# jarrodhroberson/diamond-types

Measured on AMD Instinct MI355X. Metric: merged ops/sec (whole node) for batched checkout, higher is better.
Workload: dtype u32/u8 integer

## Files before the change

diamond-types_amd/csrc/dt_device.hpp:

```cpp
#pragma once
#include <hip/hip_runtime.h>
#include <stdint.h>
#include <cstdio>

#include "dt_host.hpp"

namespace dtgpu {

inline hipError_t launch_error(const char *file = __builtin_FILE(), int line = __builtin_LINE()) {
    const hipError_t e = hipGetLastError();
    if (e != hipSuccess) fprintf(stderr, "[dtgpu] launch error at %s:%d: %s\n", file, line, hipGetErrorString(e));
    return e;
}

struct DocDesc {
    uint64_t cmd_off;
    uint64_t lv_off;
    uint64_t content_off;
    uint64_t arun_off;
    uint64_t blk_off;
    uint64_t out_off;
    uint64_t gidx_off;
    uint64_t tlist_off;
    uint32_t ncmd, n_lv, n_aruns, max_blocks, out_cap, content_len;
    uint32_t ascii;
    uint32_t seg_lo, seg_hi, seg_u, src_cap;
    uint64_t pc_off;
    uint64_t src_off;
    uint32_t flags;
};
constexpr uint32_t SEG_PHANTOM = 0x80000000u;
constexpr uint32_t DOC_CRITICAL = 1u;
constexpr uint32_t DOC_FF = 2u;
constexpr uint32_t DOC_CUT_HOST = 4u;

struct DocResult {
    uint32_t status, out_len;
    uint64_t hash;
    uint32_t n_items, n_blocks;
    uint32_t fail_cmd, fail_site;
    uint32_t n_sb, lds;
    uint32_t dbg[22];
};

constexpr uint32_t LOC_CNT_SHIFT = 24;
constexpr uint32_t LOC_BLK_SHIFT = 6;
constexpr uint32_t LOC_BLK_MASK = 0x3FFFF;
constexpr uint32_t LOC_MAX_BLOCKS = LOC_BLK_MASK + 1;

struct BatchParams {
    const Cmd *cmds;
    const uint32_t *tlist;
    const uint32_t *cbyte;
    const uint8_t *content;
    const uint32_t *aruns;
    uint32_t *pos;
    unsigned long long *ao;
    uint32_t *items;
    unsigned long long *m2;
    uint8_t *out;
    uint8_t *gidx;
    const DocDesc *docs;
    const uint32_t *doc_list;
    uint32_t n_list;
    uint32_t lds_blocks;
// ... 113 lines not shown
```

diamond-types_amd/csrc/dt_replay.hip:

```cpp
#include <hip/hip_runtime.h>

#include <algorithm>
#include <cstdlib>
#include <stdint.h>

#include "dt_device.hpp"
#include "dt_wave.hpp"

namespace dtgpu {
namespace dev {
using namespace wave;

#define BALLOT(c) __ballot(c)
DEV uint32_t vflag(bool c) {
    uint32_t x = c ? 1u : 0u;
    asm volatile("" : "+v"(x));
    return x;
}

constexpr uint32_t BLK = 64;
constexpr uint32_t SBC = 64;
constexpr uint32_t ROOT_ID = 0xFFFFFFFFu;
constexpr uint32_t END_ID = 0xFFFFFFFEu;
constexpr uint32_t NONE = 0xFFFFFFFFu;
// ... 10 lines not shown

template <typename T> DEV T ld(const T *p) { return *p; }
template <typename T> DEV T vld(const T *p) { return *reinterpret_cast<const volatile T *>(p); }
DEV const BatchParams &KP() {
    return *(const BatchParams *)(__builtin_amdgcn_kernarg_segment_ptr());
}
#define GLOBAL_AS __attribute__((address_space(1)))
template <typename T> DEV GLOBAL_AS T *gp(T *p) { return (GLOBAL_AS T *)p; }
template <typename T> DEV void st(T *p, T v) { *p = v; }
template <typename T> DEV T ld_sc(const T *p) { return __hip_atomic_load(p, __ATOMIC_RELAXED, __HIP_MEMORY_SCOPE_WORKGROUP); }
template <typename T> DEV void st_sc(T *p, T v) { __hip_atomic_store(p, v, __ATOMIC_RELAXED, __HIP_MEMORY_SCOPE_WORKGROUP); }
DEV uint32_t cv_add(uint32_t *p, uint32_t d) { return __hip_atomic_fetch_add(p, d, __ATOMIC_RELAXED, __HIP_MEMORY_SCOPE_WORKGROUP); }
template <typename T> DEV void at_xor(T *p, T v) { __hip_atomic_fetch_xor(p, v, __ATOMIC_RELAXED, __HIP_MEMORY_SCOPE_WORKGROUP); }
template <typename T> DEV void at_add(T *p, T v) { __hip_atomic_fetch_add(p, v, __ATOMIC_RELAXED, __HIP_MEMORY_SCOPE_WORKGROUP); }
template <typename T> DEV void at_or(T *p, T v) { __hip_atomic_fetch_or(p, v, __ATOMIC_RELAXED, __HIP_MEMORY_SCOPE_WORKGROUP); }

template <int L> DEV uint32_t ix(const uint32_t *p) {
    if (L) return *p;
    return ld_sc(p);
}
template <int L> DEV uint32_t ix16(const uint16_t *p) { return *p; }

enum ProfSlot { P_INS = 0, P_DEL, P_TOG, P_MAT, P_YJS, P_SPLIT, P_FIND, P_BLOAD, P_ORR, P_RUN, P_R1, P_R2, P_R3, P_N_YJS, P_N_SPLIT,
                P_T1, P_T2, P_T3, P_N_DIRTY, P_N_LOAD, P_N };

struct Doc {
    const Cmd *cmds;
    uint32_t ncmd, n_lv;
    const uint32_t *tlist;
    const DocDesc *desc;
    uint32_t *pc;
    u64 *ao;
    uint32_t *items;
    u64 *m2;
    uint32_t max_blocks, max_sb;
    uint32_t *cnt, *opos;
    uint16_t *opos16;
    uint32_t *sbn, *sbpos;
    uint32_t *top, *tlive;
    uint16_t *sbl;
    uint32_t nb, nsb;
    uint32_t err;
    uint32_t debug;
    uint32_t site;
    uint32_t steps;
    uint64_t prof[P_N];
    uint32_t doc;
    uint32_t cb, cit;
    u64 cmv, cml;
    u64 *mup;
    uint32_t *tup;
    uint32_t *xf;
};

DEV void fail(Doc &D, uint32_t code, uint32_t site) {
    if (!D.err) { D.err = code; D.site = site; }
}
DEV bool charge(Doc &D) {
    if (D.steps == 0) { fail(D, ErrCapacity, 1); return false; }
    D.steps--;
    return true;
}
template <bool PROF> DEV uint64_t tick() { return PROF ? __builtin_amdgcn_s_memtime() : 0; }

constexpr int IX_HBM = 0, IX_LDS = 1, IX_FLAT = 2;
template <int L> DEV uint32_t opos_of(const Doc &D, uint32_t b) {
    if (L) return D.opos16[b];
    return ix<L>(D.opos + b);
}
template <int L> DEV void set_opos(Doc &D, uint32_t b, uint32_t v) {
    if (L) D.opos16[b] = uint16_t(v);
    else D.opos[b] = v;
}


template <int L> DEV uint32_t first_block(const Doc &D) {
// ... 29 lines not shown
            const uint32_t o = 4 * (q + uint32_t(j));
            if (v[j].w == item) s = o + 3;
            if (v[j].z == item) s = o + 2;
            if (v[j].y == item) s = o + 1;
            if (v[j].x == item) s = o;
        }
    }
    return s;
}
template <int L> DEV uint32_t key_of(const Doc &D, uint32_t item) {
    const uint32_t b = pc_blk(ld(D.pc + item));
    return key_at<L>(D, b, find_slot(D, b, item));
}
template <int L> DEV uint32_t ukey_of(const Doc &D, uint32_t item) {
    const uint32_t b = U(pc_blk(ld(D.pc + item)));
    const u64 m = BALLOT(D.items[size_t(b) * BLK + lane()] == item);
    return U(key_at<L>(D, b, ctz(m)));
}

struct Found {
    uint32_t b, k;
    uint32_t S, tp;
    uint32_t c;
};
template <int L>
DEV bool find_vis(Doc &D, uint32_t p, Found &f) {
    const uint32_t l = lane();
    uint32_t base = 0, S = NONE;
    if (L == IX_FLAT) {
        const uint32_t nc = (D.nb + 63) >> 6;
        {
            const uint32_t w0 = D.top[min(l, nc - 1)];
            const uint32_t v = l < nc ? (w0 & 0xFFFFu) : 0u;
            const uint32_t inc = scan_incl32(v);
            const u64 m = BALLOT(inc > p) & 0xFFFFFFFFull;
            if (!m) return false;
            S = ctz(m);
            base = rdl(inc - v, S);
        }
        f.S = f.tp = S;
        const uint32_t q = (S << 6) + l;
        const uint32_t b0 = D.sbl[min(q, D.nb - 1)];
        const uint32_t w = D.cnt[b0];
        const uint32_t b = q < D.nb ? b0 : 0;
        const uint32_t v = q < D.nb ? c_vis(w) : 0;
        const uint32_t inc = scan_incl(v);
        const u64 m = BALLOT(base + inc > p);
        if (!m) return false;
        const uint32_t fl = ctz(m);
        f.b = U(rdl(b, fl));
        f.k = U(p - base - rdl(inc - v, fl));
        f.c = U(rdl(w, fl));
        return true;
    }
    for (uint32_t c = 0; c < D.nsb; c += 64) {
        const uint32_t i = c + l;
        const uint32_t w0 = ix<L>(D.top + min(i, D.nsb - 1));
        const uint32_t w = i < D.nsb ? w0 : 0;
        const uint32_t v = w & 0xFFFFu;
        const uint32_t inc = scan_incl(v);
        const u64 m = BALLOT(base + inc > p);
        if (m) {
            const uint32_t fl = ctz(m);
            S = U(rdl(w, fl) >> 16);
            f.tp = U(c + fl);
            base += rdl(inc - v, fl);
            break;
        }
        base += rdl(inc, 63);
    }
    if (S == NONE) return false;
    f.S = S;
    f.c = NONE;
    const uint32_t n = U(ix<L>(D.sbn + S));
    const uint32_t b0 = ix16<L>(D.sbl + size_t(S) * SBC + l);
// ... 206 lines not shown
    D.nb++;
    if (n + 1 == SBC) split_sb<L, XF>(D, S);
    return b2;
}

template <int L> DEV uint32_t cut_point(uint32_t s) { return L ? min(max(s, 16u), 48u) : BLK / 2; }

template <int L>
DEV uint32_t up_rank(Doc &D, uint32_t b, uint32_t s) {
    const uint32_t l = lane();
    const uint32_t o = U(opos_of<L>(D, b));
    const uint32_t S = o >> 6, i = o & 63u, tp = U(ix<L>(D.sbpos + S));
    uint32_t r = 0;
    for (uint32_t c = 0; c < tp; c += 64) r += wave_sum(c + l < tp ? ix<L>(D.tup + c + l) : 0u);
    const uint32_t bl = l < i ? ix16<L>(D.sbl + size_t(S) * SBC + l) : 0;
    r += wave_sum(l < i ? c_up(ix<L>(D.cnt + bl)) : 0u);
    r += uint32_t(__popcll(U64(ld(D.mup + b)) & lanes_below(s)));
    return U(r);
}

template <int L, bool PROF, bool XF>
DEV void insert_run(Doc &D, uint32_t b, uint32_t s, uint32_t it, u64 mv, u64 ml, uint32_t lv, uint32_t k,
                    uint32_t ol, uint32_t orr, uint32_t tph, uint32_t c_in) {
    D.cb = NONE;
    const uint32_t l = lane();
    const uint32_t lv0 = lv, k0 = k;
    if (XF) {
        const uint32_t r0 = up_rank<L>(D, b, s);
        for (uint32_t j = l; j < k0; j += 64) D.xf[lv0 + j] = r0 + j;
    }
    if (!XF && c_in != NONE && c_items(c_in) + k <= BLK) {
        const uint32_t shifted = shfl(it, l >= k ? l - k : l);
        it = l < s ? it : (l < s + k ? lv + (l - s) : shifted);
        D.items[size_t(b) * BLK + l] = it;
        if (l >= s && l < s + k) st(D.pc + it, pc_of(b, 1u));
        const u64 low = lanes_below(s);
        const u64 ins = lanes_below(k) << s;
        mv = k == 64 ? ins : ((mv & low) | ((mv & ~low) << k) | ins);
        ml = k == 64 ? ins : ((ml & low) | ((ml & ~low) << k) | ins);
        st(D.m2 + 2 * size_t(b) + (l & 1u), (l & 1u) ? ml : mv);
        if (tph == NONE) tph = L == IX_FLAT ? U(uint32_t(D.opos16[b]) >> 6) : U(ix<L>(D.sbpos + (opos_of<L>(D, b) >> 6)));
        if (l == 0) {
            D.cnt[b] = c_in + k * (C_VIS + C_LIVE + C_ITEMS);
            if (L == IX_FLAT) {
                at_add(D.top + tph, k | (k << 16));
            } else {
                at_add(D.top + tph, k);
// ... 45 lines not shown
            u64 mu = U64(ld(D.mup + b));
            mu = m == 64 ? ins : ((mu & low) | ((mu & ~low) << m) | ins);
            if (l == 0) st(D.mup + b, mu);
        }
        if (tph == NONE) tph = L == IX_FLAT ? U(uint32_t(D.opos16[b]) >> 6) : U(ix<L>(D.sbpos + (opos_of<L>(D, b) >> 6)));
        if (l == 0) {
            D.cnt[b] = c + m * (C_VIS + C_LIVE + C_ITEMS + (XF ? C_UP : 0u));
            const uint32_t tp = tph;
            if (L == IX_FLAT) {
                at_add(D.top + tp, m | (m << 16));
            } else {
                at_add(D.top + tp, m);
                at_add(D.tlive + tp, m);
            }
            if (XF) at_add(D.tup + tp, m);
        }
        fence_wave();
        if (PROF) { const uint64_t t = tick<PROF>(); D.prof[P_R2] += t - tr; tr = t; }
        lv += m;
        k -= m;
        s += m;
    }
    D.cb = b; D.cit = it; D.cmv = mv; D.cml = ml;
    const uint64_t t3 = tick<PROF>();
    for (uint32_t j0 = 0; j0 < k0; j0 += 64) {
        const uint32_t j = j0 + l, nit = lv0 + j;
        if (j < k0) D.ao[nit] = u64(j == 0 ? ol : nit - 1) | (u64(orr) << 32);
    }
    if (PROF) D.prof[P_R3] += tick<PROF>() - t3;
}

DEV void agent_of(Doc &D, uint32_t lv, uint32_t &rank, uint32_t &seq) {
    const uint32_t l = lane();
    const GLOBAL_AS uint32_t *aruns = gp(vld(&KP().aruns)) + U(uint32_t(vld(&D.desc->arun_off)));
    uint32_t lo = 0, n = U(vld(&D.desc->n_aruns));
    while (n > 64) {
        if (!charge(D)) { rank = seq = 0; return; }
        const uint32_t stride = (n + 63) / 64;
        const uint32_t idx = lo + l * stride;
        const bool ok = l * stride < n && aruns[4 * idx] <= lv;
        const uint32_t k = uint32_t(__popcll(BALLOT(ok)));
        const uint32_t nlo = lo + (k ? k - 1 : 0) * stride;
        n = min(stride, lo + n - nlo);
        lo = nlo;
    }
    const bool ok = l < n && aruns[4 * (lo + l)] <= lv;
// ... 85 lines not shown
    const uint32_t bc = c_items(c);
    if (PROF) { D.prof[P_N_LOAD]++; if (c & C_DIRTY) D.prof[P_N_DIRTY]++; }
    const uint32_t it0 = D.items[size_t(b) * BLK + l];
    it = l < bc ? it0 : 0;
    if (c & C_DIRTY) {
        const uint32_t k = pc_cnt(ld(D.pc + it));
        mv = BALLOT(l < bc && k == 1u);
        ml = BALLOT(l < bc && k != 0u);
        st(D.m2 + 2 * size_t(b) + (l & 1u), (l & 1u) ? ml : mv);
        if (l == 0) D.cnt[b] = c & ~C_DIRTY;
        fence_wave();
    } else {
        const u64 x = ld(D.m2 + 2 * size_t(b) + (l & 1u));
        mv = rdl64(x, 0);
        ml = rdl64(x, 1);
    }
}

template <int L, bool PROF, bool XF>
DEV void do_insert(Doc &D, uint32_t lv, uint32_t k, uint32_t pos) {
    uint64_t tp = tick<PROF>();
    uint32_t b, kk = 0, tph = 0;
    uint32_t fcnt = NONE;
    if (pos == 0) {
        b = first_block<L>(D);
    } else {
        Found f;
        if (!find_vis<L>(D, pos - 1, f)) { fail(D, ErrCheckout, 13); return; }
        b = f.b;
        kk = f.k;
        tph = f.tp;
        fcnt = f.c;
    }
    if (PROF) { const uint64_t t = tick<PROF>(); D.prof[P_FIND] += t - tp; tp = t; }
    const uint32_t c0 = L == IX_FLAT && fcnt != NONE ? fcnt : U(ix<L>(D.cnt + b));
    const uint32_t bc = c_items(c0);
    uint32_t cb = c0 & ~C_DIRTY;
    uint32_t it;
    u64 mv, ml;
    if (b == D.cb) { it = D.cit; mv = D.cmv; ml = D.cml; }
    else load_block<L, PROF>(D, b, c0, it, mv, ml);
    uint32_t s = 0, ol = ROOT_ID;
    if (pos) {
        const uint32_t s0 = select_bit(mv, kk);
        if (s0 >= bc) { fail(D, ErrCheckout, 13); return; }
        ol = U(rdl(it, s0));
        s = s0 + 1;
    }
    if (PROF) { const uint64_t t = tick<PROF>(); D.prof[P_BLOAD] += t - tp; tp = t; }
    const u64 mlr = s >= 64 ? 0ull : (ml & (~0ull << s));
    uint32_t rb, rs, orr;
    bool direct;
    if (mlr) {
        rb = b;
        rs = ctz(mlr);
        orr = U(rdl(it, rs));
// ... 10 lines not shown
        } else {
            rs = 0;
            orr = END_ID;
        }
        if (s < bc) direct = false;
        else {
            const uint32_t nx = next_block<L>(D, b);
            direct = nx == NONE || (rb == nx && rs == 0);
        }
    }
    if (PROF) { const uint64_t t = tick<PROF>(); D.prof[P_ORR] += t - tp; tp = t; }
    if (!direct) {
        const uint32_t my_l = ol == ROOT_ID ? 0u : ukey_of<L>(D, ol) + 1u;
        const uint32_t my_r = orr == END_ID ? 0xFFFFFFFFu : ukey_of<L>(D, orr);
        const uint32_t b0 = b;
        yjs_scan<L>(D, b, s, rb, rs, my_l, my_r, ol, orr, lv);
        if (D.err) return;
        if (b != b0) {
            cb = U(ix<L>(D.cnt + b));
            if (b == D.cb) { it = D.cit; mv = D.cmv; ml = D.cml; }
            else load_block<L, PROF>(D, b, cb, it, mv, ml);
            cb &= ~C_DIRTY;
            tph = NONE;
        }
        if (PROF) { const uint64_t t = tick<PROF>(); D.prof[P_YJS] += t - tp; tp = t; D.prof[P_N_YJS]++; }
    }
    const uint64_t sp0 = PROF ? D.prof[P_SPLIT] : 0;
    insert_run<L, PROF, XF>(D, b, s, it, mv, ml, lv, k, ol, orr, tph, cb);
    if (PROF) D.prof[P_RUN] += tick<PROF>() - tp - (D.prof[P_SPLIT] - sp0);
}

template <int L, bool PROF, bool XF>
DEV void do_delete(Doc &D, uint32_t lv, uint32_t n, uint32_t pos, bool fwd) {
    const uint32_t l = lane();
    uint32_t j0 = 0;
    uint32_t up_done = 0;
    while (j0 < n) {
        Found f;
        if (!find_vis<L>(D, pos, f)) { fail(D, ErrCheckout, 14); return; }
        const uint32_t b = f.b, kk = f.k, tpos = f.tp;
        const uint32_t c0 = L == IX_FLAT && f.c != NONE ? f.c : U(ix<L>(D.cnt + b));
        uint32_t it;
        u64 mv, ml;
        if (b == D.cb) { it = D.cit; mv = D.cmv; ml = D.cml; }
        else load_block<L, PROF>(D, b, c0, it, mv, ml);
        const uint32_t c = c0 & ~C_DIRTY;
        const uint32_t avail = c_vis(c) - kk;
        const uint32_t take = min(avail, n - j0);
        const uint32_t r = uint32_t(__popcll(mv & lanes_below(l)));
        const bool sel = ((mv >> l) & 1ull) && r >= kk && r < kk + take;
        const u64 selm = BALLOT(sel);
        if (uint32_t(__popcll(selm)) != take || take == 0) { fail(D, ErrCheckout, 15); return; }
        u64 mu = 0;
        uint32_t base = 0;
        if (XF) {
            mu = U64(ld(D.mup + b));
            base = up_rank<L>(D, b, 0);
        }
        if (sel) {
            const uint32_t j = j0 + (r - kk);
            const uint32_t dlv = fwd ? lv + j : lv + n - 1 - j;
            st(D.pc + it, pc_of(b, 2u));
// ... 85 lines not shown
                    else act = false;
                }
            }
            dm &= ~same;
        }
        bool fv = false, fl = false;
        uint32_t b = 0;
        int32_t dv = 0, dl = 0;
        {
            const uint32_t w = ld(D.pc + (act ? item : 0u));
            const uint32_t bw = pc_blk(w), oc = pc_cnt(w), nc = oc + uint32_t(d);
            const bool badc = act && int32_t((oc + uint32_t(dneg)) | (0xFFFFu - nc) | (D.nb - 1u - bw)) < 0;
            const bool ok = act && !badc;
            bad = bad || badc;
            if (ok) st(D.pc + item, pc_of(bw, nc));
            b = ok ? bw : 0u;
            fv = ok && ((oc == 1) != (nc == 1));
            fl = ok && ((oc != 0) != (nc != 0));
            dv = fv ? (nc == 1 ? 1 : -1) : 0;
            dl = fl ? (nc != 0 ? 1 : -1) : 0;
        }
        if (BALLOT(bad)) { fail(D, ErrCheckout, 16); return; }
        const bool flip = fv || fl;
        if (BALLOT(flip && b == D.cb)) D.cb = NONE;
        if (PROF) { const uint64_t t = tick<PROF>(); D.prof[P_T2] += t - tq; tq = t; }
        if (L == IX_FLAT) {
            if (flip) {
                at_add(D.top + (uint32_t(D.opos16[b]) >> 6), uint32_t(dv) + (uint32_t(dl) << 16));
                at_add(D.cnt + b, uint32_t(dv) * C_VIS + uint32_t(dl) * C_LIVE);
                at_or(D.cnt + b, C_DIRTY);
            }
        } else if (L) {
            if (flip) {
                const uint32_t tp = ix<L>(D.sbpos + (opos_of<L>(D, b) >> 6));
                if (fv) at_add(D.top + tp, uint32_t(dv));
                if (fl) at_add(D.tlive + tp, uint32_t(dl));
                at_add(D.cnt + b, uint32_t(dv) * C_VIS + uint32_t(dl) * C_LIVE);
                at_or(D.cnt + b, C_DIRTY);
            }
        } else {
            for (u64 pend = BALLOT(flip); pend;) {
                const uint32_t f = ctz(pend);
                const uint32_t bb = rdl(b, f);
                const u64 same = BALLOT(flip && b == bb);
                const bool mine = (same >> l) & 1ull;
                const uint32_t sv = wave_sum(mine ? uint32_t(dv) : 0u), sl = wave_sum(mine ? uint32_t(dl) : 0u);
                if (l == f) {
                    const uint32_t tp = ix<L>(D.sbpos + (opos_of<L>(D, bb) >> 6));
                    if (sv) at_add(D.top + tp, sv);
                    if (sl) at_add(D.tlive + tp, sl);
                    at_add(D.cnt + bb, sv * C_VIS + sl * C_LIVE);
                    at_or(D.cnt + bb, C_DIRTY);
                }
                pend &= ~same;
// ... 49 lines not shown
                const int32_t sum = int32_t(wave_sum(mine ? uint32_t(d) : 0u));
                const int32_t neg = int32_t(wave_sum(mine ? uint32_t(dneg) : 0u));
                if (mine) {
                    if (l == ctz(same)) { d = sum; dneg = neg; }
                    else act = false;
                }
            }
            dm &= ~same;
        }
    }
    if (PROF) { const uint64_t t = tick<PROF>(); D.prof[P_T1] += t - tq; tq = t; }
    const uint32_t w = ld(D.pc + (act ? item : 0u));
    const uint32_t bw = pc_blk(w), oc = pc_cnt(w), nc = oc + uint32_t(d);
    const bool badc = act && int32_t((oc + uint32_t(dneg)) | (0xFFFFu - nc) | (D.nb - 1u - bw)) < 0;
    const bool ok = act && !badc;
    if (ok) st(D.pc + item, pc_of(bw, nc));
    if (BALLOT(bad || badc)) { fail(D, ErrCheckout, 16); return; }
    const uint32_t b = ok ? bw : 0u;
    const bool fv = ok && ((oc == 1) != (nc == 1));
    const bool fl = ok && ((oc != 0) != (nc != 0));
    const int32_t dv = fv ? (nc == 1 ? 1 : -1) : 0;
    const int32_t dl = fl ? (nc != 0 ? 1 : -1) : 0;
    const bool flip = fv || fl;
    if (BALLOT(flip && b == D.cb)) D.cb = NONE;
    if (PROF) { const uint64_t t = tick<PROF>(); D.prof[P_T2] += t - tq; tq = t; }
    if (L == IX_FLAT) {
        if (flip) {
            at_add(D.top + (uint32_t(D.opos16[b]) >> 6), uint32_t(dv) + (uint32_t(dl) << 16));
            at_add(D.cnt + b, uint32_t(dv) * C_VIS + uint32_t(dl) * C_LIVE);
            at_or(D.cnt + b, C_DIRTY);
        }
    } else if (L) {
        if (flip) {
            const uint32_t tp = ix<L>(D.sbpos + (opos_of<L>(D, b) >> 6));
            if (fv) at_add(D.top + tp, uint32_t(dv));
            if (fl) at_add(D.tlive + tp, uint32_t(dl));
            at_add(D.cnt + b, uint32_t(dv) * C_VIS + uint32_t(dl) * C_LIVE);
            at_or(D.cnt + b, C_DIRTY);
        }
    } else {
        for (u64 pend = BALLOT(flip); pend;) {
            const uint32_t f = ctz(pend);
            const uint32_t bb = rdl(b, f);
            const u64 same = BALLOT(flip && b == bb);
            const bool mine = (same >> l) & 1ull;
            const uint32_t sv = wave_sum(mine ? uint32_t(dv) : 0u), sl = wave_sum(mine ? uint32_t(dl) : 0u);
            if (l == f) {
                const uint32_t tp = ix<L>(D.sbpos + (opos_of<L>(D, bb) >> 6));
                if (sv) at_add(D.top + tp, sv);
                if (sl) at_add(D.tlive + tp, sl);
                at_add(D.cnt + bb, sv * C_VIS + sl * C_LIVE);
                at_or(D.cnt + bb, C_DIRTY);
            }
            pend &= ~same;
// ... 336 lines not shown
                    if (w != b || find_slot(D, b, it) != l) bad = true;
                }
            } else if (((mv | ml) >> l) & 1) bad = true;
            const u64 bm = BALLOT(bad);
            if (bm) {
                if (l == ctz(bm)) {
                    res->dbg[0] = b; res->dbg[1] = l; res->dbg[2] = cnt; res->dbg[3] = it; res->dbg[4] = w;
                    res->dbg[5] = uint32_t(mv); res->dbg[6] = uint32_t(mv >> 32);
                    res->dbg[7] = uint32_t(ml); res->dbg[8] = uint32_t(ml >> 32);
                }
                return 202;
            }
            blocks++;
        }
        if (tv != (U(ix<L>(D.top + p)) & 0xFFFFu)) return 203;
        if (tl != (L == IX_FLAT ? U(ix<L>(D.top + p)) >> 16 : U(ix<L>(D.tlive + p)))) return 204;
        if (XF && tu != U(ix<L>(D.tup + p))) return 210;
    }
    if (blocks != D.nb) return 208;
    if (L == IX_FLAT) {
        for (uint32_t c = nlists + l; c < D.max_sb; c += 64)
            if (BALLOT(D.top[c] != 0)) return 211;
    }
    return 0;
}

template <int L, bool PROF, bool XF, bool MW>
DEV void run_doc(Doc &D) {
    const uint32_t l = lane();
    D.nb = 1;
    D.nsb = 1;
    D.err = 0;
    D.site = 0;
    const uint32_t seg_lo = U(vld(&D.desc->seg_lo)), seg_hi = U(vld(&D.desc->seg_hi));
    if (!XF && (seg_lo != 0 || seg_hi != NONE)) {
        const uint32_t c0 = seg_lo ? U(seg_cmd(D.cmds, D.ncmd, seg_lo)) : 0u;
        const uint32_t c1 = seg_hi != NONE ? U(seg_cmd(D.cmds, D.ncmd, seg_hi)) : D.ncmd;
        if (c1 < c0 || seg_straddles(D.cmds, c0, seg_lo) || seg_straddles(D.cmds, c1, seg_hi)) fail(D, ErrCheckout, 30);
        else { D.cmds += c0; D.ncmd = c1 - c0; }
    }
    D.steps = uint32_t(min<uint64_t>(64ull * (uint64_t(D.ncmd) + D.n_lv) + 4096, 0xFFFFFFF0ull));
    const uint32_t seg_u = XF ? 0u : U(vld(&D.desc->seg_u));
    if (seg_u) {
        if (!D.err) init_phantoms<L>(D, seg_u);
    } else {
        if (L == IX_FLAT) {
            for (uint32_t c = l; c < D.max_sb; c += 64) D.top[c] = 0;
            if (l == 0) { D.cnt[0] = 0; D.opos16[0] = 0; D.sbl[0] = 0; }
        } else if (l == 0) {
            D.cnt[0] = 0; set_opos<L>(D, 0, 0);
            D.sbl[0] = 0; D.sbn[0] = 1; D.sbpos[0] = 0; D.top[0] = 0; D.tlive[0] = 0;
            if (XF) { D.tup[0] = 0; st(D.mup, 0ull); }
        }
        if (l < 2) st(D.m2 + l, 0ull);
        fence_wave();
    }
    D.cb = NONE;
    D.cit = 0;
    D.cmv = D.cml = 0;
    if (PROF) for (int i = 0; i < P_N; i++) D.prof[i] = 0;
    const uint64_t t_start = tick<PROF>();
    uint32_t pf = 0;
    bool pf_ok = false;
    uint32_t ci = 0;
    for (uint32_t base = 0; base < D.ncmd && !D.err; base += 64) {
        const uint32_t n_here = min(64u, D.ncmd - base);
        Cmd pre = {0, 0, 0, 0};
        pre = D.cmds[min(base + l, D.ncmd - 1)];
        const uint32_t op_l = pre.op & 15u;
        const bool apply_l = op_l == CMD_INS || op_l == CMD_DEL;
        const u64 bad_cmds = BALLOT(l < n_here && (op_l > CMD_TOG || (apply_l && (pre.len == 0 || pre.lv >= D.n_lv ||
                                                                               pre.len > D.n_lv - pre.lv))));
        const u64 tog_cmds = BALLOT(l < n_here && op_l == CMD_TOG);
        const uint32_t n_ok = bad_cmds ? ctz(bad_cmds) : n_here;
        for (uint32_t j = 0; j < n_ok && !D.err; j++) {
            ci = base + j;
            const uint32_t op = U(rdl(pre.op, j)), a = U(rdl(pre.lv, j)), n = U(rdl(pre.len, j)),
                           pos = U(rdl(pre.pos, j));
            uint32_t nx_pf = 0;
            bool nx_ok = false;
            if ((tog_cmds >> j) & 2ull) {
                const uint32_t o2 = U(rdl(pre.lv, j + 1)), n2 = U(rdl(pre.len, j + 1));
// ... 44 lines not shown
        } else {
            GLOBAL_AS uint8_t *out = gp(vld(&KP().out)) + vld(&D.desc->out_off);
            materialise<L>(D, out, U(vld(&D.desc->out_cap)), len, h, n_items);
        }
    }
    GLOBAL_AS DocResult *res = gp(vld(&KP().results)) + D.doc;
    if (l == 0) {
        res->status = D.err;
        res->out_len = len;
        res->hash = h;
        res->n_items = n_items;
        res->n_blocks = D.nb;
        res->n_sb = D.nsb;
        res->lds = L ? 1u : 0u;
        res->fail_cmd = D.err ? ci : 0;
        res->fail_site = D.err ? D.site : 0;
        if (PROF && (D.debug & 2u)) {
            D.prof[P_MAT] = tick<PROF>() - t_mat;
            for (int i = 0; i < P_T1; i++) res->dbg[i] = uint32_t(D.prof[i] >> (i < P_N_YJS ? 4 : 0));
            res->dbg[15] = uint32_t((tick<PROF>() - t_start) >> 4);
            for (int i = P_T1; i < P_N_DIRTY; i++) res->dbg[16 + (i - P_T1)] = uint32_t(D.prof[i] >> 4);
            res->dbg[19] = uint32_t(D.prof[P_N_DIRTY]);
            res->dbg[20] = uint32_t(D.prof[P_N_LOAD]);
        }
    }
}

DEV void bind_index(Doc &D, uint8_t *base, uint32_t mb, uint32_t ms, bool narrow) {
    uint32_t *w = reinterpret_cast<uint32_t *>(base);
    D.cnt = w; w += mb;
    if (narrow) { D.opos16 = reinterpret_cast<uint16_t *>(w); D.opos = nullptr; w += (mb + 1) / 2; }
    else { D.opos = w; D.opos16 = nullptr; w += mb; }
    D.top = w; w += ms;
    D.tlive = w; w += ms;
    D.sbn = w; w += ms;
    D.sbpos = w; w += ms;
    D.sbl = reinterpret_cast<uint16_t *>(w);
}

DEV void bind_index_flat(Doc &D, uint8_t *base, uint32_t mb) {
    uint32_t *w = reinterpret_cast<uint32_t *>(base);
    D.cnt = w; w += mb;
    D.opos16 = reinterpret_cast<uint16_t *>(w); w += (mb + 1) / 2;
    D.sbl = reinterpret_cast<uint16_t *>(w); w += (mb + 1) / 2;
    D.top = w;
    D.opos = D.tlive = D.sbn = D.sbpos = nullptr;
// ... 225 lines not shown
```

diamond-types_amd/csrc/dtgpu_pass.cpp:

```cpp
#include <cstdio>
#include <cstring>

#include "dt_batch.hpp"
#include "dt_merge.hpp"

using namespace dtgpu;

namespace {

int wait_for(hipStream_t s, hipEvent_t e) { return hipStreamWaitEvent(s, e, 0) == hipSuccess ? OK : ErrHip; }
int hop(hipEvent_t e, hipStream_t from, hipStream_t to) {
    return hipEventRecord(e, from) == hipSuccess ? wait_for(to, e) : ErrHip;
}

struct Pipe {
    PrepParams prep;
    PlanParams plan;
    CutParams cut;
    hipStream_t s, w;
    hipEvent_t w0, w1, cut_done;
};
Pipe whole_pipe(const dtgpu_batch *B, hipStream_t s) {
    return Pipe{B->prep, B->plan, B->cut, s, B->wstream, B->ev_w0, B->ev_w1, B->ev_cut};
}
// ... 458 lines not shown
        hipStreamSynchronize(B->stream) != hipSuccess)
        return DTGPU_ERR_HIP;
    for (int k = 0; k < 6; k++) out[k] = r.prof[k];
    out[6] = r.ncmd;
    out[7] = r.ntlist;
    return DTGPU_OK;
}
dtgpu_status dtgpu_batch_doc_stats(dtgpu_batch *B, size_t i, uint32_t out[29]) {
    if (!B || i >= B->docs.size() || !out) return DTGPU_ERR_ARG;
    DocResult r;
    if (hipMemcpyAsync(&r, B->d_results.p + i, sizeof r, hipMemcpyDeviceToHost, B->stream) != hipSuccess ||
        hipStreamSynchronize(B->stream) != hipSuccess)
        return DTGPU_ERR_HIP;
    out[0] = r.n_items; out[1] = r.n_blocks; out[2] = r.fail_cmd; out[3] = r.fail_site;
    out[4] = B->docs[i].ncmd; out[5] = B->docs[i].max_blocks;
    for (int k = 0; k < 16; k++) out[6 + k] = r.dbg[k];
    out[22] = r.n_sb;
    out[23] = r.lds;
    for (int k = 0; k < 3; k++) out[24 + k] = r.dbg[16 + k];
    out[27] = r.dbg[19];
    out[28] = r.dbg[20];
    return DTGPU_OK;
}
uint64_t dtgpu_batch_total_lv(const dtgpu_batch *B) { return B ? B->total_lv : 0; }

dtgpu_status dtgpu_batch_results(dtgpu_batch *B, dtgpu_doc_result *res) {
    if (!B || (!res && B->n)) return DTGPU_ERR_ARG;
    std::vector<DocResult> dr(B->n);
    if (B->n && hipMemcpyAsync(dr.data(), B->d_results.p, B->n * sizeof(DocResult), hipMemcpyDeviceToHost, B->stream) != hipSuccess)
        return DTGPU_ERR_HIP;
    if (hipStreamSynchronize(B->stream) != hipSuccess) return DTGPU_ERR_HIP;
    for (size_t i = 0; i < B->n; i++) {
        res[i].status = B->host_status[i] != OK ? B->host_status[i] : dr[i].status;
        res[i].reserved = 0;
        res[i].text_len = res[i].status == OK ? dr[i].out_len : 0;
        res[i].text_hash = res[i].status == OK ? dr[i].hash : 0;
        res[i].n_lv = B->n_lv[i];
    }
    return DTGPU_OK;
}
dtgpu_status dtgpu_batch_text(dtgpu_batch *B, size_t i, uint8_t *out, size_t cap, size_t *out_len) {
    if (!B || i >= B->n) return DTGPU_ERR_ARG;
    if (B->host_status[i] != OK) return dtgpu_status(B->host_status[i]);
    DocResult r;
    if (hipMemcpyAsync(&r, B->d_results.p + i, sizeof r, hipMemcpyDeviceToHost, B->stream) != hipSuccess ||
        hipStreamSynchronize(B->stream) != hipSuccess)
// ... 20 lines not shown
```

diamond-types_amd/dt_amd/__init__.py:

```python
import collections
import ctypes
import os

_HERE = os.path.dirname(os.path.abspath(__file__))
LIB_PATH = os.path.join(os.path.dirname(_HERE), os.environ.get("DTGPU_LIB_DIR", "lib"), "libdtgpu.so")

STATUS_NAMES = {
    0: "OK", 1: "InvalidMagic", 2: "UnsupportedProtocolVersion", 3: "DocIdMismatch", 4: "BaseVersionUnknown",
    5: "UnknownChunk", 6: "LZ4DecoderNeeded", 7: "LZ4DecompressionError", 8: "CompressedDataMissing",
    9: "InvalidChunkHeader", 10: "MissingChunk", 11: "InvalidLength", 12: "UnexpectedEOF", 13: "InvalidUTF8",
    14: "InvalidRemoteID", 15: "InvalidVarInt", 16: "InvalidContent", 17: "GenericInvalidData",
    18: "ChecksumFailed", 19: "DataMissing", 64: "ErrCheckout", 65: "ErrCapacity", 66: "ErrHip", 67: "ErrArg",
    68: "ErrNoDevice",
}


class ParseError(Exception):

    def __init__(self, code):
        self.code = code
        self.name = STATUS_NAMES.get(code, str(code))
        super().__init__(f"{self.name} ({code})")


# ... 120 lines not shown
    L.dtgpu_oplog_doc_id.argtypes = [vp, ctypes.c_char_p, sz]
    L.dtgpu_oplog_doc_id.restype = ctypes.c_int64
    L.dtgpu_oplog_set_doc_id.argtypes = [vp, ctypes.c_char_p, sz]
    L.dtgpu_xf_operations.argtypes = [vp, ctypes.POINTER(ctypes.c_uint32), sz, ctypes.POINTER(sz)]
    L.dtgpu_oplog_xf_order.argtypes = [vp, pu64, sz, pu64, sz, ctypes.POINTER(ctypes.c_uint32), sz]
    L.dtgpu_oplog_xf_order.restype = sz
    L.dtgpu_xf_operations_from.argtypes = [vp, pu64, sz, pu64, sz, ctypes.POINTER(ctypes.c_uint32), sz,
                                           ctypes.POINTER(sz)]
    L.dtgpu_batch_create.argtypes = [ctypes.POINTER(ctypes.c_char_p), ctypes.POINTER(sz), sz,
                                     ctypes.POINTER(BatchOpts), ctypes.POINTER(vp)]
    L.dtgpu_batch_create_from_oplogs.argtypes = [ctypes.POINTER(vp), sz, ctypes.POINTER(BatchOpts), ctypes.POINTER(vp)]
    L.dtgpu_batch_create_xf.argtypes = [ctypes.POINTER(vp), sz, ctypes.POINTER(BatchOpts), ctypes.POINTER(vp)]
    L.dtgpu_batch_xf_positions.argtypes = [vp, sz, ctypes.POINTER(ctypes.c_uint32), sz, ctypes.POINTER(sz)]
    L.dtgpu_batch_run.argtypes = [vp, vp]
    L.dtgpu_batch_run_timed.argtypes = [vp, ctypes.POINTER(ctypes.c_float)]
    L.dtgpu_batch_sync.argtypes = [vp]
    L.dtgpu_batch_size.argtypes = [vp]
    L.dtgpu_batch_size.restype = sz
    L.dtgpu_batch_results.argtypes = [vp, ctypes.POINTER(DocResult)]
    L.dtgpu_batch_text.argtypes = [vp, sz, ctypes.c_char_p, sz, ctypes.POINTER(sz)]
    L.dtgpu_batch_algorithmic_bytes.argtypes = [vp]
    L.dtgpu_batch_algorithmic_bytes.restype = u64
    L.dtgpu_batch_doc_stats.argtypes = [vp, sz, ctypes.POINTER(ctypes.c_uint32)]
    L.dtgpu_batch_segments.argtypes = [vp, sz, ctypes.POINTER(ctypes.c_uint32), sz]
    L.dtgpu_batch_segments.restype = sz
    L.dtgpu_oplog_cut_ranges.argtypes = [vp, ctypes.POINTER(ctypes.c_uint64), sz]
    L.dtgpu_oplog_cut_ranges.restype = sz
    L.dtgpu_batch_plan_profile.argtypes = [vp, sz, ctypes.POINTER(ctypes.c_uint64)]
    L.dtgpu_batch_total_lv.argtypes = [vp]
    L.dtgpu_batch_total_lv.restype = u64
    L.dtgpu_batch_free.argtypes = [vp]
    L.dtgpu_batch_create_device.argtypes = [ctypes.POINTER(ctypes.c_char_p), ctypes.POINTER(sz), sz,
                                            ctypes.POINTER(BatchOpts), ctypes.POINTER(vp)]
    L.dtgpu_batch_run_e2e_timed.argtypes = [vp, ctypes.POINTER(ctypes.c_float)]
    L.dtgpu_batch_encode.argtypes = [vp, ctypes.c_uint32, ctypes.POINTER(ctypes.c_float)]
    L.dtgpu_batch_encoded.argtypes = [vp, sz, ctypes.c_char_p, sz, ctypes.POINTER(sz), ctypes.POINTER(ctypes.c_uint64)]
    L.dtgpu_batch_encoded_bytes.argtypes = [vp, ctypes.c_int]
    L.dtgpu_batch_encoded_bytes.restype = ctypes.c_uint64
    L.dtgpu_batch_checkout.argtypes = [ctypes.POINTER(ctypes.c_char_p), ctypes.POINTER(sz), sz,
                                       ctypes.POINTER(BatchOpts), ctypes.POINTER(DocResult)]
    L.dtgpu_text_hash.argtypes = [ctypes.c_char_p, sz]
    L.dtgpu_text_hash.restype = u64
    L.dtgpu_device_count.restype = c
    L.dtgpu_synth_ops.argtypes = [u64, ctypes.c_uint32, ctypes.POINTER(ctypes.c_uint32), ctypes.POINTER(ctypes.c_uint32), sz]
    L.dtgpu_synth_ops.restype = sz
    L.dtgpu_synth_oplog.argtypes = [u64, ctypes.c_uint32, ctypes.POINTER(vp)]
# ... 687 lines not shown
        return [int(x) for x in buf[:n]]

    def plan(self, i):
        nc, nt = ctypes.c_size_t(), ctypes.c_size_t()
        _check(lib().dtgpu_batch_plan(self._h, i, None, 0, None, 0, ctypes.byref(nc), ctypes.byref(nt)))
        cb = (ctypes.c_uint32 * max(4, 4 * nc.value))()
        tb = (ctypes.c_uint32 * max(1, nt.value))()
        _check(lib().dtgpu_batch_plan(self._h, i, cb, nc.value, tb, nt.value, ctypes.byref(nc), ctypes.byref(nt)))
        return [tuple(cb[4 * k:4 * k + 4]) for k in range(nc.value)], list(tb[:nt.value])

    def plan_profile(self, i):
        out = (ctypes.c_uint64 * 8)()
        _check(lib().dtgpu_batch_plan_profile(self._h, i, out))
        keys = ["rec", "parents", "children", "emit", "ops", "init", "n_cmds", "n_tlist"]
        return dict(zip(keys, list(out)))

    def doc_stats(self, i):
        out = (ctypes.c_uint32 * 29)()
        _check(lib().dtgpu_batch_doc_stats(self._h, i, out))
        keys = ["n_items", "n_blocks", "fail_cmd", "fail_site", "n_cmds", "max_blocks",
                "cyc_ins", "cyc_del", "cyc_tog", "cyc_mat", "cyc_yjs", "cyc_split", "cyc_find", "cyc_bload",
                "cyc_orr", "cyc_run", "cyc_r1", "cyc_r2", "cyc_r3", "n_yjs", "n_split", "cyc_total",
                "n_sb", "lds_index", "cyc_t1", "cyc_t2", "cyc_t3", "n_dirty", "n_load"]
        return dict(zip(keys, list(out)))

    def segments(self, i):
        out = (ctypes.c_uint32 * (12 * 64))()
        n = lib().dtgpu_batch_segments(self._h, i, out, 64)
        keys = ["lo", "hi", "placeholders", "status", "items_visible", "cyc_total", "lds_index", "n_blocks",
                "host_fallback", "host_lo", "host_hi", "host_placeholders"]
        return [dict(zip(keys, list(out[12 * k:12 * k + 12]))) for k in range(min(n, 64))]

    @property
    def algorithmic_bytes(self):
        return lib().dtgpu_batch_algorithmic_bytes(self._h)

    @property
    def total_lv(self):
        return lib().dtgpu_batch_total_lv(self._h)


class DecodeBatch:

    def __init__(self, docs, ignore_crc=False, device=0):
        L = lib()
        n = len(docs)
        self._keep = [bytes(d) for d in docs]
# ... 446 lines not shown
```

include/dtgpu.h:

```cpp
#ifndef DTGPU_H
#define DTGPU_H

#include <stddef.h>
#include <stdint.h>

#ifdef __cplusplus
extern "C" {
#endif

typedef enum dtgpu_status {
    DTGPU_OK = 0,
    DTGPU_INVALID_MAGIC = 1,
    DTGPU_UNSUPPORTED_PROTOCOL_VERSION = 2,
    DTGPU_DOC_ID_MISMATCH = 3,
    DTGPU_BASE_VERSION_UNKNOWN = 4,
    DTGPU_UNKNOWN_CHUNK = 5,
    DTGPU_LZ4_DECODER_NEEDED = 6,
    DTGPU_LZ4_DECOMPRESSION_ERROR = 7,
    DTGPU_COMPRESSED_DATA_MISSING = 8,
    DTGPU_INVALID_CHUNK_HEADER = 9,
    DTGPU_MISSING_CHUNK = 10,
    DTGPU_INVALID_LENGTH = 11,
    DTGPU_UNEXPECTED_EOF = 12,
    DTGPU_INVALID_UTF8 = 13,
// ... 120 lines not shown
    uint64_t text_len;
    uint64_t text_hash;
    uint64_t n_lv;
} dtgpu_doc_result;

dtgpu_status dtgpu_batch_create(const uint8_t *const *docs, const size_t *lens, size_t n_docs,
                                const dtgpu_batch_opts *opts, dtgpu_batch **out);
dtgpu_status dtgpu_batch_create_from_oplogs(const dtgpu_oplog *const *oplogs, size_t n_docs,
                                            const dtgpu_batch_opts *opts, dtgpu_batch **out);
dtgpu_status dtgpu_batch_run(dtgpu_batch *batch, void *stream);
dtgpu_status dtgpu_batch_run_timed(dtgpu_batch *batch, float *kernel_ms);
dtgpu_status dtgpu_batch_sync(dtgpu_batch *batch);
size_t dtgpu_batch_size(const dtgpu_batch *batch);
dtgpu_status dtgpu_batch_last_times(const dtgpu_batch *batch, float out[3]);
size_t dtgpu_batch_host_planned(const dtgpu_batch *batch, uint8_t *flags, size_t cap);
size_t dtgpu_batch_fast_forwarded(const dtgpu_batch *batch, uint8_t *flags, size_t cap);
size_t dtgpu_batch_late_pipelined(const dtgpu_batch *batch, uint8_t *flags, size_t cap);
dtgpu_status dtgpu_batch_plan(dtgpu_batch *batch, size_t doc, uint32_t *cmds, size_t cmd_cap, uint32_t *tlist,
                              size_t tlist_cap, size_t *n_cmds, size_t *n_tlist);
dtgpu_status dtgpu_batch_results(dtgpu_batch *batch, dtgpu_doc_result *results);
dtgpu_status dtgpu_batch_text(dtgpu_batch *batch, size_t doc, uint8_t *out, size_t cap, size_t *out_len);
uint64_t dtgpu_batch_algorithmic_bytes(dtgpu_batch *batch);
dtgpu_status dtgpu_batch_doc_stats(dtgpu_batch *batch, size_t doc, uint32_t out[29]);
size_t dtgpu_batch_segments(dtgpu_batch *batch, size_t doc, uint32_t *out, size_t cap);
dtgpu_status dtgpu_batch_plan_profile(dtgpu_batch *batch, size_t doc, uint64_t out[8]);
uint64_t dtgpu_batch_total_lv(const dtgpu_batch *batch);
void dtgpu_batch_free(dtgpu_batch *batch);

dtgpu_status dtgpu_batch_checkout(const uint8_t *const *docs, const size_t *lens, size_t n_docs,
                                  const dtgpu_batch_opts *opts, dtgpu_doc_result *results);

uint64_t dtgpu_text_hash(const uint8_t *text, size_t len);

dtgpu_status dtgpu_batch_create_xf(const dtgpu_oplog *const *oplogs, size_t n_docs, const dtgpu_batch_opts *opts,
                                   dtgpu_batch **out);
dtgpu_status dtgpu_batch_xf_positions(dtgpu_batch *batch, size_t doc, uint32_t *out, size_t cap, size_t *n_out);


size_t dtgpu_synth_ops(uint64_t doc, uint32_t target_ops, uint32_t *n_agents, uint32_t *out, size_t cap);
dtgpu_status dtgpu_synth_oplog(uint64_t doc, uint32_t target_ops, dtgpu_oplog **out);
dtgpu_status dtgpu_synth_merge_oplog(uint64_t doc, uint32_t target_ops, uint32_t n_agents, dtgpu_oplog **out);

int dtgpu_device_count(void);
const char *dtgpu_status_str(dtgpu_status status);


// ... 105 lines not shown
```

Measured before the change: 9.994 billion.

## Cache visible-prefix rank of current block to skip position lookups

```diff
diff --git a/diamond-types_amd/csrc/dt_device.hpp b/diamond-types_amd/csrc/dt_device.hpp
--- a/diamond-types_amd/csrc/dt_device.hpp
+++ b/diamond-types_amd/csrc/dt_device.hpp
@@ -40,7 +40,7 @@
     uint32_t n_items, n_blocks;
     uint32_t fail_cmd, fail_site;
     uint32_t n_sb, lds;
-    uint32_t dbg[22];
+    uint32_t dbg[24];
 };
 
 constexpr uint32_t LOC_CNT_SHIFT = 24;
diff --git a/diamond-types_amd/csrc/dt_replay.hip b/diamond-types_amd/csrc/dt_replay.hip
--- a/diamond-types_amd/csrc/dt_replay.hip
+++ b/diamond-types_amd/csrc/dt_replay.hip
@@ -56,7 +56,7 @@
 template <int L> DEV uint32_t ix16(const uint16_t *p) { return *p; }
 
 enum ProfSlot { P_INS = 0, P_DEL, P_TOG, P_MAT, P_YJS, P_SPLIT, P_FIND, P_BLOAD, P_ORR, P_RUN, P_R1, P_R2, P_R3, P_N_YJS, P_N_SPLIT,
-                P_T1, P_T2, P_T3, P_N_DIRTY, P_N_LOAD, P_N };
+                P_T1, P_T2, P_T3, P_N_DIRTY, P_N_LOAD, P_N_LOOK, P_N_SKIP, P_N };
 
 struct Doc {
     const Cmd *cmds;
@@ -82,10 +82,14 @@
     uint32_t doc;
     uint32_t cb, cit;
     u64 cmv, cml;
+    uint32_t cpre, cpos;
     u64 *mup;
     uint32_t *tup;
     uint32_t *xf;
 };
+
+constexpr uint32_t PRE_NONE = 0x80000000u;
+DEV bool pre_known(uint32_t pre) { return int32_t(pre) >= 0; }
 
 DEV void fail(Doc &D, uint32_t code, uint32_t site) {
     if (!D.err) { D.err = code; D.site = site; }
@@ -161,6 +165,7 @@
     uint32_t b, k;
     uint32_t S, tp;
     uint32_t c;
+    uint32_t p;
 };
 template <int L>
 DEV bool find_vis(Doc &D, uint32_t p, Found &f) {
@@ -190,6 +195,7 @@
         f.b = U(rdl(b, fl));
         f.k = U(p - base - rdl(inc - v, fl));
         f.c = U(rdl(w, fl));
+        f.p = (S << 6) + fl;
         return true;
     }
     for (uint32_t c = 0; c < D.nsb; c += 64) {
@@ -442,7 +448,9 @@
 template <int L, bool PROF, bool XF>
 DEV void insert_run(Doc &D, uint32_t b, uint32_t s, uint32_t it, u64 mv, u64 ml, uint32_t lv, uint32_t k,
                     uint32_t ol, uint32_t orr, uint32_t tph, uint32_t c_in) {
+    constexpr bool PC = L == IX_FLAT && !XF;
     D.cb = NONE;
+    const uint32_t b_in = b;
     const uint32_t l = lane();
     const uint32_t lv0 = lv, k0 = k;
     if (XF) {
@@ -534,6 +542,7 @@
         s += m;
     }
     D.cb = b; D.cit = it; D.cmv = mv; D.cml = ml;
+    if (PC && b != b_in) D.cpre = PRE_NONE;
     const uint64_t t3 = tick<PROF>();
     for (uint32_t j0 = 0; j0 < k0; j0 += 64) {
         const uint32_t j = j0 + l, nit = lv0 + j;
@@ -665,16 +674,29 @@
     uint64_t tp = tick<PROF>();
     uint32_t b, kk = 0, tph = 0;
     uint32_t fcnt = NONE;
+    constexpr bool PC = L == IX_FLAT && !XF;
     if (pos == 0) {
         b = first_block<L>(D);
+        if (PC) { D.cpre = 0; D.cpos = 0; }
     } else {
-        Found f;
-        if (!find_vis<L>(D, pos - 1, f)) { fail(D, ErrCheckout, 13); return; }
-        b = f.b;
-        kk = f.k;
-        tph = f.tp;
-        fcnt = f.c;
-    }
+        const uint32_t rk = pos - 1 - D.cpre;
+        const uint32_t hit = PC ? U(uint32_t(rk < uint32_t(__popcll(D.cmv)))) : 0u;
+        if (hit) {
+            b = D.cb;
+            kk = rk;
+            tph = D.cpos >> 6;
+        } else {
+            Found f;
+            if (!find_vis<L>(D, pos - 1, f)) { fail(D, ErrCheckout, 13); return; }
+            b = f.b;
+            kk = f.k;
+            tph = f.tp;
+            fcnt = f.c;
+            if (PC) { D.cpre = pos - 1 - f.k; D.cpos = f.p; }
+        }
+        if (PC && PROF) D.prof[P_N_SKIP] += hit;
+    }
+    if (PC && PROF) D.prof[P_N_LOOK]++;
     if (PROF) { const uint64_t t = tick<PROF>(); D.prof[P_FIND] += t - tp; tp = t; }
     const uint32_t c0 = L == IX_FLAT && fcnt != NONE ? fcnt : U(ix<L>(D.cnt + b));
     const uint32_t bc = c_items(c0);
@@ -731,6 +753,7 @@
             else load_block<L, PROF>(D, b, cb, it, mv, ml);
             cb &= ~C_DIRTY;
             tph = NONE;
+            if (PC) D.cpre = PRE_NONE;
         }
         if (PROF) { const uint64_t t = tick<PROF>(); D.prof[P_YJS] += t - tp; tp = t; D.prof[P_N_YJS]++; }
     }
@@ -745,8 +768,20 @@
     uint32_t j0 = 0;
     uint32_t up_done = 0;
     while (j0 < n) {
+        constexpr bool PC = L == IX_FLAT && !XF;
         Found f;
-        if (!find_vis<L>(D, pos, f)) { fail(D, ErrCheckout, 14); return; }
+        const uint32_t rk = pos - D.cpre;
+        const uint32_t hit = PC ? U(uint32_t(rk < uint32_t(__popcll(D.cmv)))) : 0u;
+        if (hit) {
+            f.b = D.cb;
+            f.k = rk;
+            f.tp = D.cpos >> 6;
+            f.c = NONE;
+        } else {
+            if (!find_vis<L>(D, pos, f)) { fail(D, ErrCheckout, 14); return; }
+            if (PC) { D.cpre = pos - f.k; D.cpos = f.p; }
+        }
+        if (PC && PROF) { D.prof[P_N_LOOK]++; D.prof[P_N_SKIP] += hit; }
         const uint32_t b = f.b, kk = f.k, tpos = f.tp;
         const uint32_t c0 = L == IX_FLAT && f.c != NONE ? f.c : U(ix<L>(D.cnt + b));
         uint32_t it;
@@ -878,14 +913,17 @@
         }
         if (BALLOT(bad)) { fail(D, ErrCheckout, 16); return; }
         const bool flip = fv || fl;
-        if (BALLOT(flip && b == D.cb)) D.cb = NONE;
+        if (BALLOT(flip && b == D.cb)) { D.cb = NONE; if (L == IX_FLAT) D.cpre = PRE_NONE; }
         if (PROF) { const uint64_t t = tick<PROF>(); D.prof[P_T2] += t - tq; tq = t; }
         if (L == IX_FLAT) {
+            uint32_t pb = NONE;
             if (flip) {
-                at_add(D.top + (uint32_t(D.opos16[b]) >> 6), uint32_t(dv) + (uint32_t(dl) << 16));
+                pb = D.opos16[b];
+                at_add(D.top + (pb >> 6), uint32_t(dv) + (uint32_t(dl) << 16));
                 at_add(D.cnt + b, uint32_t(dv) * C_VIS + uint32_t(dl) * C_LIVE);
                 at_or(D.cnt + b, C_DIRTY);
             }
+            if (pre_known(D.cpre)) D.cpre += U(wave_sum(pb < D.cpos ? uint32_t(dv) : 0u));
         } else if (L) {
             if (flip) {
                 const uint32_t tp = ix<L>(D.sbpos + (opos_of<L>(D, b) >> 6));
@@ -981,14 +1019,17 @@
     const int32_t dv = fv ? (nc == 1 ? 1 : -1) : 0;
     const int32_t dl = fl ? (nc != 0 ? 1 : -1) : 0;
     const bool flip = fv || fl;
-    if (BALLOT(flip && b == D.cb)) D.cb = NONE;
+    if (BALLOT(flip && b == D.cb)) { D.cb = NONE; if (L == IX_FLAT) D.cpre = PRE_NONE; }
     if (PROF) { const uint64_t t = tick<PROF>(); D.prof[P_T2] += t - tq; tq = t; }
     if (L == IX_FLAT) {
+        uint32_t pb = NONE;
         if (flip) {
-            at_add(D.top + (uint32_t(D.opos16[b]) >> 6), uint32_t(dv) + (uint32_t(dl) << 16));
+            pb = D.opos16[b];
+            at_add(D.top + (pb >> 6), uint32_t(dv) + (uint32_t(dl) << 16));
             at_add(D.cnt + b, uint32_t(dv) * C_VIS + uint32_t(dl) * C_LIVE);
             at_or(D.cnt + b, C_DIRTY);
         }
+        if (pre_known(D.cpre)) D.cpre += U(wave_sum(pb < D.cpos ? uint32_t(dv) : 0u));
     } else if (L) {
         if (flip) {
             const uint32_t tp = ix<L>(D.sbpos + (opos_of<L>(D, b) >> 6));
@@ -1371,6 +1412,16 @@
         for (uint32_t c = nlists + l; c < D.max_sb; c += 64)
             if (BALLOT(D.top[c] != 0)) return 211;
     }
+    if (L == IX_FLAT && !XF && D.cb != NONE && pre_known(D.cpre)) {
+        if (D.cb >= D.nb || U(D.opos16[D.cb]) != D.cpos) return 212;
+        uint32_t before = 0;
+        for (uint32_t q0 = 0; q0 < D.cpos; q0 += 64) {
+            const uint32_t q = q0 + l;
+            before += wave_sum(q < D.cpos ? c_vis(D.cnt[D.sbl[min(q, D.nb - 1)]]) : 0u);
+        }
+        if (U(before) != D.cpre) return 212;
+        if (uint32_t(__popcll(D.cmv)) != c_vis(U(D.cnt[D.cb]))) return 213;
+    }
     return 0;
 }
 
@@ -1407,6 +1458,8 @@
     D.cb = NONE;
     D.cit = 0;
     D.cmv = D.cml = 0;
+    D.cpre = PRE_NONE;
+    D.cpos = 0;
     if (PROF) for (int i = 0; i < P_N; i++) D.prof[i] = 0;
     const uint64_t t_start = tick<PROF>();
     uint32_t pf = 0;
@@ -1497,6 +1550,8 @@
             for (int i = P_T1; i < P_N_DIRTY; i++) res->dbg[16 + (i - P_T1)] = uint32_t(D.prof[i] >> 4);
             res->dbg[19] = uint32_t(D.prof[P_N_DIRTY]);
             res->dbg[20] = uint32_t(D.prof[P_N_LOAD]);
+            res->dbg[21] = uint32_t(D.prof[P_N_LOOK]);
+            res->dbg[22] = uint32_t(D.prof[P_N_SKIP]);
         }
     }
 }
diff --git a/diamond-types_amd/csrc/dtgpu_pass.cpp b/diamond-types_amd/csrc/dtgpu_pass.cpp
--- a/diamond-types_amd/csrc/dtgpu_pass.cpp
+++ b/diamond-types_amd/csrc/dtgpu_pass.cpp
@@ -504,6 +504,16 @@
     out[28] = r.dbg[20];
     return DTGPU_OK;
 }
+dtgpu_status dtgpu_batch_lookup_stats(dtgpu_batch *B, size_t i, uint32_t out[2]) {
+    if (!B || i >= B->docs.size() || !out) return DTGPU_ERR_ARG;
+    DocResult r;
+    if (hipMemcpyAsync(&r, B->d_results.p + i, sizeof r, hipMemcpyDeviceToHost, B->stream) != hipSuccess ||
+        hipStreamSynchronize(B->stream) != hipSuccess)
+        return DTGPU_ERR_HIP;
+    out[0] = r.dbg[21];
+    out[1] = r.dbg[22];
+    return DTGPU_OK;
+}
 uint64_t dtgpu_batch_total_lv(const dtgpu_batch *B) { return B ? B->total_lv : 0; }
 
 dtgpu_status dtgpu_batch_results(dtgpu_batch *B, dtgpu_doc_result *res) {
diff --git a/diamond-types_amd/dt_amd/__init__.py b/diamond-types_amd/dt_amd/__init__.py
--- a/diamond-types_amd/dt_amd/__init__.py
+++ b/diamond-types_amd/dt_amd/__init__.py
@@ -166,6 +166,7 @@
     L.dtgpu_batch_algorithmic_bytes.argtypes = [vp]
     L.dtgpu_batch_algorithmic_bytes.restype = u64
     L.dtgpu_batch_doc_stats.argtypes = [vp, sz, ctypes.POINTER(ctypes.c_uint32)]
+    L.dtgpu_batch_lookup_stats.argtypes = [vp, sz, ctypes.POINTER(ctypes.c_uint32)]
     L.dtgpu_batch_segments.argtypes = [vp, sz, ctypes.POINTER(ctypes.c_uint32), sz]
     L.dtgpu_batch_segments.restype = sz
     L.dtgpu_oplog_cut_ranges.argtypes = [vp, ctypes.POINTER(ctypes.c_uint64), sz]
@@ -899,7 +900,11 @@
                 "cyc_ins", "cyc_del", "cyc_tog", "cyc_mat", "cyc_yjs", "cyc_split", "cyc_find", "cyc_bload",
                 "cyc_orr", "cyc_run", "cyc_r1", "cyc_r2", "cyc_r3", "n_yjs", "n_split", "cyc_total",
                 "n_sb", "lds_index", "cyc_t1", "cyc_t2", "cyc_t3", "n_dirty", "n_load"]
-        return dict(zip(keys, list(out)))
+        st = dict(zip(keys, list(out)))
+        look = (ctypes.c_uint32 * 2)()
+        _check(lib().dtgpu_batch_lookup_stats(self._h, i, look))
+        st["n_lookup"], st["n_lookup_skip"] = look[0], look[1]
+        return st
 
     def segments(self, i):
         out = (ctypes.c_uint32 * (12 * 64))()
diff --git a/include/dtgpu.h b/include/dtgpu.h
--- a/include/dtgpu.h
+++ b/include/dtgpu.h
@@ -166,6 +166,7 @@
 dtgpu_status dtgpu_batch_text(dtgpu_batch *batch, size_t doc, uint8_t *out, size_t cap, size_t *out_len);
 uint64_t dtgpu_batch_algorithmic_bytes(dtgpu_batch *batch);
 dtgpu_status dtgpu_batch_doc_stats(dtgpu_batch *batch, size_t doc, uint32_t out[29]);
+dtgpu_status dtgpu_batch_lookup_stats(dtgpu_batch *batch, size_t doc, uint32_t out[2]);
 size_t dtgpu_batch_segments(dtgpu_batch *batch, size_t doc, uint32_t *out, size_t cap);
 dtgpu_status dtgpu_batch_plan_profile(dtgpu_batch *batch, size_t doc, uint64_t out[8]);
 uint64_t dtgpu_batch_total_lv(const dtgpu_batch *batch);
```

After: 10.14 billion (median of 6 runs). +1.5%, better.
